# Reecepbcups/celestia-app

Hardware: AMD Instinct MI355X
Metric: ODS→EDS+DAH blocks/sec at k=128 (1/8 GPU); achieved HBM GB/s (higher is better)
Workload: dtype u8; 1 GPU; k128_block_batch: da.ExtendShares+NewDataAvailabilityHeader on 128 independent k=128 blocks per GPU per step (configs[1] per block, batched as configs[2]); k=128, parallelism=blocks x1

## Files before the change

celestia-app_amd/csrc/nmt_dev.h:

```cpp
#pragma once
#include <hip/hip_runtime.h>
#include <stdint.h>

#include "cda_internal.h"
#include "sha256_dev.h"

namespace cda {

__device__ __forceinline__ void load16(const uint4* p, uint32_t* w) {
#pragma unroll
  for (int i = 0; i < 4; i++) {
    uint4 v = p[i];
    w[4 * i + 0] = v.x;
    w[4 * i + 1] = v.y;
    w[4 * i + 2] = v.z;
    w[4 * i + 3] = v.w;
  }
}

__device__ __forceinline__ int ns_cmp(const uint32_t* a, const uint32_t* b) {
#pragma unroll
  for (int i = 0; i < 8; i++) {
    uint32_t x = bswap(a[i]), y = bswap(b[i]);
    if (i == 7) {
      x >>= 24;
      y >>= 24;
    }
    if (x != y) return x < y ? -1 : 1;
  }
  return 0;
}

constexpr uint32_t kParityLeafMid7[8] = {0x1ca5c518, 0x33e5c969, 0xbd2d00ce, 0xa4502bae,
                                         0xce23fa11, 0x90a5b516, 0x5df56d75, 0xf3f677da};
#ifndef CDA_NO_PARITY_MID
#define CDA_NO_PARITY_MID 0
#endif

template <bool PAIRS = true>
__device__ __forceinline__ void leaf_record(const uint4* sh, uint32_t* A, bool q0, uint4* out) {
  uint32_t N[16];
  if (PAIRS) load16(sh + 4, N);
  uint32_t ns[8];
#pragma unroll
  for (int i = 0; i < 8; i++) ns[i] = q0 ? A[i] : 0xFFFFFFFFu;
  uint32_t st[8];
  sha256_init(st);
  uint32_t m[16];
  if (q0) {
    m[0] = be_window(0u, A[0], 3);
#pragma unroll
    for (int i = 1; i < 7; i++) m[i] = be_window(A[i - 1], A[i], 3);
    m[7] = (be_window(A[6], A[7], 3) & 0xFFFF0000u) | (bswap(A[0]) >> 16);
  } else {
    m[0] = 0x00FFFFFFu;
#pragma unroll
    for (int i = 1; i < 7; i++) m[i] = 0xFFFFFFFFu;
    m[7] = 0xFFFF0000u | (bswap(A[0]) >> 16);
  }
#pragma unroll
  for (int i = 8; i < 16; i++) m[i] = be_window(A[i - 8], A[i - 7], 2);
  if (!CDA_NO_PARITY_MID && __all(!q0)) {
    uint32_t mw[16], mid[8];
    mw[0] = 0x00FFFFFFu;
#pragma unroll
    for (int i = 1; i < 7; i++) mw[i] = 0xFFFFFFFFu;
#pragma unroll
    for (int i = 7; i < 16; i++) mw[i] = m[i];
#pragma unroll
    for (int i = 0; i < 8; i++) mid[i] = kParityLeafMid7[i];
    sha256_compress_fenced_from<7, false>(st, mid, mw);
  } else {
    sha256_compress(st, m);
  }
  uint32_t H[8];
#pragma unroll
  for (int i = 0; i < 8; i++) H[i] = A[8 + i];
#pragma unroll 1
  for (int j = 1; j < 8; j++) {
    uint32_t C[16];
    if (!PAIRS) {
      load16(sh + 4 * j, C);
    } else if (j & 1) {
#pragma unroll
      for (int i = 0; i < 16; i++) C[i] = N[i];
    } else {
      load16(sh + 4 * j, C);
      load16(sh + 4 * (j + 1), N);
    }
#pragma unroll
    for (int i = 0; i < 7; i++) m[i] = be_window(H[i], H[i + 1], 2);
    m[7] = be_window(H[7], C[0], 2);
#pragma unroll
    for (int i = 8; i < 16; i++) m[i] = be_window(C[i - 8], C[i - 7], 2);
    sha256_compress(st, m);
#pragma unroll
    for (int i = 0; i < 8; i++) H[i] = C[8 + i];
  }
#pragma unroll
  for (int i = 0; i < 7; i++) m[i] = be_window(H[i], H[i + 1], 2);
  m[7] = be_window(H[7], 0x80u, 2);
#pragma unroll
  for (int i = 8; i < 15; i++) m[i] = 0;
  m[15] = 542u * 8u;
  sha256_compress(st, m);
  uint32_t d[8];
#pragma unroll
  for (int i = 0; i < 8; i++) d[i] = bswap(st[i]);
  uint32_t o[24];
#pragma unroll
  for (int i = 0; i < 7; i++) o[i] = ns[i];
  o[7] = (ns[7] & 0xFFu) | (ns[0] << 8);
#pragma unroll
  for (int i = 8; i < 14; i++) o[i] = le_window(ns[i - 8], ns[i - 7], 3);
  o[14] = (le_window(ns[6], ns[7], 3) & 0xFFFFu) | (d[0] << 16);
#pragma unroll
  for (int i = 15; i < 22; i++) o[i] = le_window(d[i - 15], d[i - 14], 2);
  o[22] = d[7] >> 16;
  o[23] = 0;
#pragma unroll
  for (int i = 0; i < 6; i++) out[i] = make_uint4(o[4 * i], o[4 * i + 1], o[4 * i + 2], o[4 * i + 3]);
}

__device__ __forceinline__ void leaf_cell(const uint8_t* __restrict__ eds, uint4* __restrict__ nodes,
                                          unsigned long long* __restrict__ status, int k, int log2w, uint32_t gid) {
  const int w = 1 << log2w;
  const uint32_t cell = gid & ((1u << (2 * log2w)) - 1);
  const uint32_t blk = gid >> (2 * log2w);
  const int r = (int)(cell >> log2w), c = (int)(cell & (w - 1));
  const bool q0 = (r < k) && (c < k);
  const uint4* sh = reinterpret_cast<const uint4*>(eds + (size_t)gid * CDA_SHARE);

  uint32_t A[16];
  load16(sh, A);
  uint32_t ns[8];
#pragma unroll
  for (int i = 0; i < 8; i++) ns[i] = A[i];

  if (q0) {
    if (c + 1 < k) {
      uint32_t nb[8];
      const uint4* p = reinterpret_cast<const uint4*>(eds + ((size_t)gid + 1) * CDA_SHARE);
      uint4 v0 = p[0], v1 = p[1];
      nb[0] = v0.x; nb[1] = v0.y; nb[2] = v0.z; nb[3] = v0.w;
      nb[4] = v1.x; nb[5] = v1.y; nb[6] = v1.z; nb[7] = v1.w;
      if (ns_cmp(nb, ns) < 0) {
        unsigned long long key = ((unsigned long long)CDA_AXIS_ROW << 40) | ((unsigned long long)r << 20) | (c + 1);
        atomicMin(status + blk, key);
      }
    }
    if (r + 1 < k) {
      uint32_t nb[8];
      const uint4* p = reinterpret_cast<const uint4*>(eds + ((size_t)gid + w) * CDA_SHARE);
      uint4 v0 = p[0], v1 = p[1];
      nb[0] = v0.x; nb[1] = v0.y; nb[2] = v0.z; nb[3] = v0.w;
      nb[4] = v1.x; nb[5] = v1.y; nb[6] = v1.z; nb[7] = v1.w;
      if (ns_cmp(nb, ns) < 0) {
        unsigned long long key = ((unsigned long long)CDA_AXIS_COL << 40) | ((unsigned long long)c << 20) | (r + 1);
        atomicMin(status + blk, key);
      }
    }
  }

  leaf_record(sh, A, q0, nodes + (size_t)gid * 6);
}

__device__ __forceinline__ void ld4(const uint4* p, uint32_t* w) {
#pragma unroll
  for (int i = 0; i < 4; i++) {
    const uint4 v = p[i];
    w[4 * i + 0] = v.x;
    w[4 * i + 1] = v.y;
    w[4 * i + 2] = v.z;
    w[4 * i + 3] = v.w;
  }
}

constexpr uint32_t kParityMid14[8] = {0xa8abd42b, 0x092979bd, 0x8d5926ca, 0x8df58526,
                                      0xa812caa9, 0x7cc8da5d, 0x33a85111, 0x7d669380};
__device__ __forceinline__ void hash_node_mem(const uint4* pl, const uint4* pr, uint4* po, bool store = true,
                                              uint4* ns_lds = nullptr, bool parity = false) {
  uint32_t st[8], m[16];
  sha256_init(st);
  {
    uint32_t L[16];
    ld4(launder(pl), L);
    m[0] = be_window(0x01000000u, L[0], 3);
#pragma unroll
    for (int i = 1; i < 16; i++) m[i] = be_window(L[i - 1], L[i], 3);
    if (ns_lds)
#pragma unroll
      for (int i = 0; i < 4; i++) ns_lds[i] = make_uint4(L[4 * i], L[4 * i + 1], L[4 * i + 2], L[4 * i + 3]);
  }
  if (__all(parity)) {
    uint32_t mw[16];
    mw[0] = 0x01FFFFFFu;
#pragma unroll
    for (int i = 1; i < 14; i++) mw[i] = 0xFFFFFFFFu;
    mw[14] = m[14];
    mw[15] = m[15];
    uint32_t mid[8];
#pragma unroll
    for (int i = 0; i < 8; i++) mid[i] = kParityMid14[i];
    sha256_compress_fenced_from<14>(st, mid, mw);
  } else {
    sha256_compress_fenced(st, m);
  }
  {
    uint32_t L[16], R[16];
    ld4(launder_after(pl, st[0]) + 3, L);
    ld4(launder_after(pr, st[0]), R);
    if (ns_lds)
#pragma unroll
      for (int i = 0; i < 4; i++) ns_lds[4 + i] = make_uint4(R[4 * i], R[4 * i + 1], R[4 * i + 2], R[4 * i + 3]);
#pragma unroll
    for (int i = 0; i < 16; i++) {
      const int wi = 16 + i;
      if (wi <= 21) m[i] = be_window(L[wi - 13], L[wi - 12], 3);
      else if (wi == 22) m[i] = be_window(L[9], L[10], 3) | (R[0] & 0xFFu);
      else m[i] = be_window(R[wi - 23], R[wi - 22], 1);
    }
  }
  sha256_compress_fenced(st, m);
  {
    uint32_t R[16];
    ld4(launder_after(pr, st[0]) + 2, R);
#pragma unroll
    for (int i = 0; i < 16; i++) {
      const int wi = 32 + i;
      if (wi <= 44) m[i] = be_window(R[wi - 31], R[wi - 30], 1);
      else if (wi == 45) m[i] = be_window(R[14], R[15], 1) | 0x00800000u;
      else if (wi == 46) m[i] = 0;
      else m[i] = 181u * 8u;
    }
  }
  sha256_compress_fenced(st, m);

  uint32_t L[16], R[16];
  if (ns_lds) {
    uint32_t z = 0;
    asm volatile("" : "+v"(z) : "v"(st[0]));
    ld4(ns_lds + z, L);
    ld4(ns_lds + z + 4, R);
#pragma unroll
    for (int i = 0; i < 16; i++) asm volatile("" : "+v"(L[i]), "+v"(R[i]));
  } else {
    ld4(launder_after(pl, st[0]), L);
    ld4(launder_after(pr, st[0]), R);
  }
  bool rmin_max = true;
#pragma unroll
  for (int i = 0; i < 7; i++) rmin_max &= (R[i] == 0xFFFFFFFFu);
  rmin_max &= ((R[7] & 0xFFu) == 0xFFu);
  uint32_t S[16];
#pragma unroll
  for (int i = 7; i < 15; i++) S[i] = rmin_max ? L[i] : R[i];
  uint32_t d[8];
#pragma unroll
  for (int i = 0; i < 8; i++) d[i] = bswap(st[i]);
  uint32_t o[24];
#pragma unroll
  for (int i = 0; i < 7; i++) o[i] = L[i];
  o[7] = (L[7] & 0xFFu) | (S[7] & 0xFFFFFF00u);
#pragma unroll
  for (int i = 8; i < 14; i++) o[i] = S[i];
  o[14] = (S[14] & 0xFFFFu) | (d[0] << 16);
#pragma unroll
  for (int i = 15; i < 22; i++) o[i] = le_window(d[i - 15], d[i - 14], 2);
  o[22] = d[7] >> 16;
  o[23] = 0;
  if (store)
#pragma unroll
    for (int i = 0; i < 6; i++) po[i] = make_uint4(o[4 * i], o[4 * i + 1], o[4 * i + 2], o[4 * i + 3]);
}

template <int B>
__device__ __forceinline__ void node_block(const uint32_t (&L)[24], const uint32_t (&R)[24], uint32_t (&m)[16]) {
#pragma unroll
  for (int i = 0; i < 16; i++) {
    const int wi = 16 * B + i;
    if (wi == 0) m[i] = be_window(0x01000000u, L[0], 3);
    else if (wi <= 21) m[i] = be_window(L[wi - 1], L[wi], 3);
    else if (wi == 22) m[i] = be_window(L[21], L[22], 3) | (R[0] & 0xFFu);
    else if (wi <= 44) m[i] = be_window(R[wi - 23], R[wi - 22], 1);
    else if (wi == 45) m[i] = be_window(R[22], R[23], 1) | 0x00800000u;
    else if (wi == 46) m[i] = 0;
    else m[i] = 181u * 8u;
  }
}
__device__ __forceinline__ void node_record(const uint32_t (&L)[24], const uint32_t (&R)[24], const uint32_t (&st)[8],
                                            uint32_t (&o)[24]);

__device__ __forceinline__ void hash_node_regs(const uint32_t (&L)[24], const uint32_t (&R)[24], uint32_t (&o)[24]) {
  uint32_t st[8], m[16];
  sha256_init(st);
  node_block<0>(L, R, m);
  sha256_compress(st, m);
  node_block<1>(L, R, m);
  sha256_compress(st, m);
  node_block<2>(L, R, m);
  sha256_compress(st, m);
  node_record(L, R, st, o);
}
__device__ __forceinline__ void node_record(const uint32_t (&L)[24], const uint32_t (&R)[24], const uint32_t (&st)[8],
                                            uint32_t (&o)[24]) {
  bool rmin_max = true;
#pragma unroll
  for (int i = 0; i < 7; i++) rmin_max &= (R[i] == 0xFFFFFFFFu);
  rmin_max &= ((R[7] & 0xFFu) == 0xFFu);
  uint32_t S[16];
#pragma unroll
  for (int i = 7; i < 15; i++) S[i] = rmin_max ? L[i] : R[i];
  uint32_t d[8];
#pragma unroll
  for (int i = 0; i < 8; i++) d[i] = bswap(st[i]);
#pragma unroll
  for (int i = 0; i < 7; i++) o[i] = L[i];
  o[7] = (L[7] & 0xFFu) | (S[7] & 0xFFFFFF00u);
#pragma unroll
  for (int i = 8; i < 14; i++) o[i] = S[i];
  o[14] = (S[14] & 0xFFFFu) | (d[0] << 16);
#pragma unroll
  for (int i = 15; i < 22; i++) o[i] = le_window(d[i - 15], d[i - 14], 2);
  o[22] = d[7] >> 16;
  o[23] = 0;
}

}
```

celestia-app_amd/csrc/nmt_kernels.hip:

```cpp
#include <hip/hip_runtime.h>
#include <stdint.h>
#include <stdlib.h>

#include <algorithm>
#include <cstdio>
#include <cstdlib>
#include <mutex>
#include <set>

#include "cda_internal.h"
#include "nmt_dev.h"
#include "sha256_dev.h"

namespace cda {

__global__ void __launch_bounds__(256) leaf_hash_kernel(const uint8_t* __restrict__ eds, uint4* __restrict__ nodes,
                                                        unsigned long long* __restrict__ status, int k, int log2w,
                                                        uint32_t total_cells) {
  const uint32_t gid = blockIdx.x * blockDim.x + threadIdx.x;
  if (gid >= total_cells) return;
  leaf_cell(eds, nodes, status, k, log2w, gid);
}

__device__ __forceinline__ void load_node(const uint4* p, uint32_t* n) {
#pragma unroll
  for (int i = 0; i < 6; i++) {
    uint4 v = p[i];
    n[4 * i + 0] = v.x;
    n[4 * i + 1] = v.y;
    n[4 * i + 2] = v.z;
    n[4 * i + 3] = v.w;
  }
}

template <bool FROM_LEAVES>
__global__ void __launch_bounds__(256) nmt_level_kernel(const uint4* __restrict__ in, uint4* __restrict__ out,
                                                        int log2w, int log2n_out, uint32_t total_out) {
  uint32_t gid = blockIdx.x * blockDim.x + threadIdx.x;
  if (gid >= total_out) return;
  const int w = 1 << log2w;
  const uint32_t j = gid & ((1u << log2n_out) - 1);
  const uint32_t tree_g = gid >> log2n_out;
  const uint32_t blk = tree_g >> (log2w + 1);
  const uint32_t tree = tree_g & (2 * w - 1);
  size_t ia, ib;
  if (FROM_LEAVES) {
    const size_t base = (size_t)blk << (2 * log2w);
    if (tree < (uint32_t)w) {
      ia = base + ((size_t)tree << log2w) + 2 * j;
      ib = ia + 1;
    } else {
      const uint32_t col = tree - w;
      ia = base + ((size_t)(2 * j) << log2w) + col;
      ib = ia + w;
    }
  } else {
    ia = ((size_t)tree_g << (log2n_out + 1)) + 2 * j;
    ib = ia + 1;
  }
  hash_node_mem(in + ia * 6, in + ib * 6, out + (size_t)gid * 6);
}

struct LevelDesc {
  uint4* p;
  unsigned long long blk;
  unsigned row0, row_t, row_i, col0, col_t, col_i;
};
struct LevelSet {
  LevelDesc lv[4];
};

__device__ __forceinline__ uint4* level_rec(const LevelDesc& d, unsigned b, bool col, unsigned tree, unsigned i) {
  const unsigned long long off =
      (unsigned long long)b * d.blk + (col ? d.col0 + tree * d.col_t + i * d.col_i : d.row0 + tree * d.row_t + i * d.row_i);
  return d.p + off * 6;
}

__global__ void __launch_bounds__(256) nmt_levels_kernel(LevelSet ls, int log2w, int log2n_out, int M, uint32_t total) {
  const uint32_t gid = blockIdx.x * blockDim.x + threadIdx.x;
  if (gid >= total) return;
  const unsigned w = 1u << log2w;
  const unsigned per_kind = w << log2n_out;
  const unsigned b = gid / (2 * per_kind);
  const unsigned rem = gid - b * 2 * per_kind;
  const bool col = rem >= per_kind;
  const unsigned r2 = col ? rem - per_kind : rem;
  const unsigned tree = col ? (r2 & (w - 1)) : (r2 >> log2n_out);
  const unsigned j = col ? (r2 >> log2w) : (r2 & ((1u << log2n_out) - 1));
  __shared__ uint4 s_ns[256 * 8];
  const unsigned k = w >> 1;
  const int l_in = log2w - log2n_out - M;
  for (int q = 1; q <= M; q++) {
    const unsigned cnt = 1u << (M - q);
    for (unsigned t = 0; t < cnt; t++) {
      const unsigned i = j * cnt + t;
#if CDA_NO_PARITY_MID
      const bool parity = false;
#else
      const bool parity = tree >= k || (i << (l_in + q)) >= k;
#endif
      hash_node_mem(level_rec(ls.lv[q - 1], b, col, tree, 2 * i), level_rec(ls.lv[q - 1], b, col, tree, 2 * i + 1),
                    level_rec(ls.lv[q], b, col, tree, i), true, s_ns + threadIdx.x * 8, parity);
    }
    if (q < M) asm volatile("s_waitcnt vmcnt(0)" ::: "memory");
  }
}

int launch_nmt_trees(const void* d_leaves, void* d_levels, void* d_roots, int k, int nblocks, hipStream_t s,
                     void* prof_ctx) {
  const int w = 2 * k;
  int L = 0;
  while ((1 << L) < w) L++;
  if ((1 << L) != w || L < 1) return -2;
  auto desc = [&](int l) {
    LevelDesc d{};
    const unsigned n = (unsigned)(w >> l);
    if (l == 0) {
      d.p = (uint4*)d_leaves;
      d.blk = (unsigned long long)w * w;
      d.row0 = 0, d.row_t = w, d.row_i = 1, d.col0 = 0, d.col_t = 1, d.col_i = w;
    } else if (l == L) {
      d.p = (uint4*)d_roots;
      d.blk = 2ull * w;
      d.row0 = 0, d.row_t = 1, d.row_i = 0, d.col0 = w, d.col_t = 1, d.col_i = 0;
    } else {
      unsigned long long off = 0;
      for (int q = 1; q < l; q++) off += 2ull * w * (w >> q);
      d.p = (uint4*)d_levels + off * (unsigned long long)nblocks * 6;
      d.blk = 2ull * w * n;
      d.row0 = 0, d.row_t = n, d.row_i = 1, d.col0 = w * n, d.col_t = 1, d.col_i = w;
    }
    return d;
  };
  for (int l_in = 0; l_in < L;) {
    int M = std::min(2, L - l_in);
    if (L - l_in == 3) M = 3;
    LevelSet ls{};
    for (int q = 0; q <= M; q++) ls.lv[q] = desc(l_in + q);
    const int log2n_out = L - (l_in + M);
    const uint32_t total = (uint32_t)nblocks * 2u * ((uint32_t)w << log2n_out);
    {
      ProfScope ps(prof_ctx, l_in == 0 ? "nmt_levels_1" : "nmt_levels", s);
      hipLaunchKernelGGL(nmt_levels_kernel, dim3((total + 255) / 256), dim3(256), 0, s, ls, L, log2n_out, M, total);
    }
    if (hipGetLastError() != hipSuccess) return -1;
    l_in += M;
  }
  return 0;
}

template <int B>
__device__ __forceinline__ void dah_leaf_block(const uint32_t (&L)[24], uint32_t (&m)[16]) {
#pragma unroll
  for (int t = 0; t < 16; t++) {
    const int wi = 16 * B + t;
    if (wi == 0) m[t] = be_window(0u, L[0], 3);
    else if (wi <= 21) m[t] = be_window(L[wi - 1], L[wi], 3);
    else if (wi == 22) m[t] = be_window(L[21], L[22], 3) | 0x80u;
    else if (wi < 31) m[t] = 0;
    else m[t] = 91u * 8u;
  }
}
__device__ __forceinline__ void dah_leaf_digest(const uint32_t (&L)[24], uint32_t (&st)[8]) {
  uint32_t m[16];
  sha256_init(st);
  dah_leaf_block<0>(L, m);
  sha256_compress(st, m);
  dah_leaf_block<1>(L, m);
  sha256_compress(st, m);
}
template <int B>
__device__ __forceinline__ void rfc_node_block(const uint32_t* Ld, const uint32_t* Rd, uint32_t (&m)[16]) {
  if (B == 0) {
    m[0] = 0x01000000u | (Ld[0] >> 8);
#pragma unroll
    for (int t = 1; t < 8; t++) m[t] = (Ld[t - 1] << 24) | (Ld[t] >> 8);
    m[8] = (Ld[7] << 24) | (Rd[0] >> 8);
#pragma unroll
    for (int t = 9; t < 16; t++) m[t] = (Rd[t - 9] << 24) | (Rd[t - 8] >> 8);
  } else {
    m[0] = (Rd[7] << 24) | 0x00800000u;
#pragma unroll
    for (int t = 1; t < 15; t++) m[t] = 0;
    m[15] = 65u * 8u;
  }
}

__device__ __forceinline__ void dah_fold_kw(uint32_t* sdig, int n, uint32_t* out, uint32_t* kw) {
  uint32_t* src = sdig;
  uint32_t* dst = sdig + n * 8;
  for (int cnt = n; cnt > 1;) {
    const int out_cnt = (cnt + 1) >> 1;
    if (out_cnt > 64) {
      for (int i = threadIdx.x; i < out_cnt; i += blockDim.x) {
        uint32_t* o = dst + i * 8;
        const uint32_t* Ld = src + (2 * i) * 8;
        if (2 * i + 1 >= cnt) {
#pragma unroll
          for (int t = 0; t < 8; t++) o[t] = Ld[t];
          continue;
        }
        const uint32_t* Rd = src + (2 * i + 1) * 8;
        uint32_t st[8], m[16];
        sha256_init(st);
        rfc_node_block<0>(Ld, Rd, m);
        sha256_compress(st, m);
        rfc_node_block<1>(Ld, Rd, m);
        sha256_compress(st, m);
#pragma unroll
        for (int t = 0; t < 8; t++) o[t] = st[t];
      }
    } else {
      const int i = threadIdx.x & 63;
      const bool pair = i < out_cnt && 2 * i + 1 < cnt;
      uint32_t st[8];
      if (threadIdx.x < 64) {
        const uint32_t* Ld = src + (2 * i) * 8;
        if (i < out_cnt && !pair)
#pragma unroll
          for (int t = 0; t < 8; t++) dst[i * 8 + t] = Ld[t];
        uint32_t m[16];
        sha256_init(st);
        rfc_node_block<0>(Ld, src + (2 * i + 1) * 8, m);
        sha256_compress(st, m);
      } else if (threadIdx.x < 128) {
        uint32_t m[16];
        rfc_node_block<1>(src + (2 * i) * 8, src + (2 * i + 1) * 8, m);
        sha256_kw_store(m, kw + i * kKwStride);
      }
      __syncthreads();
      if (threadIdx.x < 64) {
        sha256_rounds_kw(st, kw + i * kKwStride);
        if (pair)
#pragma unroll
          for (int t = 0; t < 8; t++) dst[i * 8 + t] = st[t];
      }
    }
    __syncthreads();
    uint32_t* tmp = src;
    src = dst;
    dst = tmp;
    cnt = out_cnt;
  }
  if (threadIdx.x < 8) out[threadIdx.x] = bswap(src[threadIdx.x]);
}

__global__ void __launch_bounds__(256) dah_kernel(const uint4* __restrict__ roots, uint32_t* __restrict__ dah,
                                                  int n) {
  extern __shared__ __attribute__((aligned(16))) uint32_t sdig[];
  const uint4* rb = roots + (size_t)blockIdx.x * n * 6;
  for (int i = threadIdx.x; i < n; i += blockDim.x) {
    uint32_t L[24], st[8];
    load_node(rb + (size_t)i * 6, L);
    dah_leaf_digest(L, st);
#pragma unroll
    for (int t = 0; t < 8; t++) sdig[i * 8 + t] = st[t];
  }
  __syncthreads();
  dah_fold_kw(sdig, n, dah + blockIdx.x * 8, sdig + (n + (n + 1) / 2) * 8);
}

__global__ void __launch_bounds__(256) dah_wide_kernel(const uint4* __restrict__ roots, uint32_t* __restrict__ dah,
                                                       unsigned* __restrict__ done, uint32_t* __restrict__ digests,
                                                       int n, int P) {
  extern __shared__ __attribute__((aligned(16))) uint32_t sdig[];
  __shared__ unsigned last;
  const unsigned b = blockIdx.x / P, part = blockIdx.x % P;
  if (threadIdx.x == 0) last = 0;
  const int i = part * 256 + threadIdx.x;
  if (i < n) {
    uint32_t L[24], st[8];
    load_node(roots + ((size_t)b * n + i) * 6, L);
    dah_leaf_digest(L, st);
    uint4* dg = reinterpret_cast<uint4*>(digests + ((size_t)b * n + i) * 8);
    dg[0] = make_uint4(st[0], st[1], st[2], st[3]);
    dg[1] = make_uint4(st[4], st[5], st[6], st[7]);
  }
  __threadfence();
  __syncthreads();
  if (threadIdx.x == 0) {
    const unsigned prev = __hip_atomic_fetch_add(done + b, 1u, __ATOMIC_ACQ_REL, __HIP_MEMORY_SCOPE_AGENT);
    if (prev == (unsigned)P - 1) last = 1;
  }
  __syncthreads();
  if (!last) return;
  __atomic_thread_fence(__ATOMIC_ACQUIRE);
  const uint4* src = reinterpret_cast<const uint4*>(digests + (size_t)b * n * 8);
  for (int x = threadIdx.x; x < n * 2; x += blockDim.x) reinterpret_cast<uint4*>(sdig)[x] = src[x];
  __syncthreads();
  dah_fold_kw(sdig, n, dah + b * 8, sdig + (n + (n + 1) / 2) * 8);
  if (threadIdx.x == 0) __hip_atomic_store(done + b, 0u, __ATOMIC_RELAXED, __HIP_MEMORY_SCOPE_AGENT);
}

constexpr int kLdsRec = 7;
#ifndef CDA_TREES_TRACE
#define CDA_TREES_TRACE 0
#endif
#if CDA_TREES_TRACE
__device__ unsigned long long* g_trees_trace;
#endif
struct TreesStamps {
  unsigned long long* v;
};
__device__ __forceinline__ void trees_mark(TreesStamps& ts, int slot) {
#if CDA_TREES_TRACE
  if (threadIdx.x == 0) {
    ts.v[2 * slot] = __builtin_amdgcn_s_memrealtime();
    ts.v[2 * slot + 1] = __builtin_amdgcn_s_memtime();
  }
#else
  (void)ts, (void)slot;
#endif
}
__device__ __forceinline__ void trees_flush(const TreesStamps& ts, int lo, int hi) {
#if CDA_TREES_TRACE
  if (threadIdx.x == 0 && g_trees_trace)
    for (int s = lo; s < hi; s++) {
      g_trees_trace[((size_t)blockIdx.x * 32 + s) * 2] = ts.v[2 * s];
      g_trees_trace[((size_t)blockIdx.x * 32 + s) * 2 + 1] = ts.v[2 * s + 1];
    }
#else
  (void)ts, (void)lo, (void)hi;
#endif
}
__device__ __forceinline__ void load_pair(const uint4* in, int i, uint32_t (&L)[24], uint32_t (&R)[24]) {
#pragma unroll
  for (int q = 0; q < 6; q++) {
    const uint4 u = in[(2 * i) * kLdsRec + q], v = in[(2 * i + 1) * kLdsRec + q];
    L[4 * q] = u.x, L[4 * q + 1] = u.y, L[4 * q + 2] = u.z, L[4 * q + 3] = u.w;
    R[4 * q] = v.x, R[4 * q + 1] = v.y, R[4 * q + 2] = v.z, R[4 * q + 3] = v.w;
  }
}
__global__ void __launch_bounds__(256) trees_lds_kernel(const uint4* __restrict__ leaves, uint4* __restrict__ roots,
                                                        uint32_t* __restrict__ dah, unsigned* __restrict__ done,
                                                        uint32_t* __restrict__ digests, int log2w) {
  extern __shared__ __attribute__((aligned(16))) uint4 lds[];
  __shared__ unsigned last;
  const int w = 1 << log2w, n = 2 * w;
  const int half = threadIdx.x >> 7, ht = threadIdx.x & 127;
  const unsigned gtree = blockIdx.x * 2 + half;
  const unsigned b = gtree >> (log2w + 1), tree = gtree & (n - 1);
  const bool col = tree >= (unsigned)w;
  const unsigned t = tree & (w - 1);
  const uint4* lb = leaves + (size_t)b * w * w * 6;
#if CDA_TREES_TRACE
  __shared__ unsigned long long tstamp[64];
  TreesStamps tst{tstamp};
#else
  TreesStamps tst{nullptr};
#endif
  trees_mark(tst, 0);
  if (threadIdx.x == 0) last = 0;
  uint4* A = lds + (size_t)half * (w + w / 2) * kLdsRec;
  uint4* B = A + (size_t)w * kLdsRec;
  uint32_t* kw = reinterpret_cast<uint32_t*>(lds + (size_t)2 * (w + w / 2 + 1) * kLdsRec) + half * 2 * 64 * kKwStride;
  for (int x = ht; x < w * 6; x += 128) {
    const int i = x / 6, q = x - i * 6;
    const size_t rec = col ? ((size_t)i << log2w) + t : ((size_t)t << log2w) + i;
    A[i * kLdsRec + q] = lb[rec * 6 + q];
  }
  __syncthreads();
  trees_mark(tst, 1);
  for (int l = 1; l <= log2w; l++) {
    const uint4* in = (l & 1) ? A : B;
    uint4* out = (l & 1) ? B : A;
    const int nodes = w >> l;
    if (nodes > 64) {
      for (int i = ht; i < nodes; i += 128) {
        uint32_t L[24], R[24], o[24];
        load_pair(in, i, L, R);
        hash_node_regs(L, R, o);
#pragma unroll
        for (int q = 0; q < 6; q++) out[i * kLdsRec + q] = make_uint4(o[4 * q], o[4 * q + 1], o[4 * q + 2], o[4 * q + 3]);
      }
    } else {
      const int i = ht & 63;
      uint32_t L[24], R[24], st[8];
      load_pair(in, i, L, R);
      if (ht < 64) {
        uint32_t m[16];
        sha256_init(st);
        node_block<0>(L, R, m);
        sha256_compress(st, m);
        trees_mark(tst, 2 + 3 * (l - 1));
      } else {
        uint32_t m[16];
        node_block<1>(L, R, m);
        sha256_kw_store(m, kw + i * kKwStride);
        node_block<2>(L, R, m);
        sha256_kw_store(m, kw + (64 + i) * kKwStride);
      }
      __syncthreads();
      trees_mark(tst, 3 + 3 * (l - 1));
      if (ht < 64) {
        sha256_rounds_kw(st, kw + i * kKwStride);
        sha256_rounds_kw(st, kw + (64 + i) * kKwStride);
        uint32_t o[24];
        node_record(L, R, st, o);
        if (i < nodes)
#pragma unroll
          for (int q = 0; q < 6; q++)
            out[i * kLdsRec + q] = make_uint4(o[4 * q], o[4 * q + 1], o[4 * q + 2], o[4 * q + 3]);
      }
    }
    __syncthreads();
// ... 587 lines not shown
```

celestia-app_amd/csrc/sha256_dev.h:

```cpp
#pragma once
#include <hip/hip_runtime.h>
#include <stdint.h>

namespace cda {

__device__ __forceinline__ uint32_t rotr(uint32_t x, int n) { return __builtin_amdgcn_alignbit(x, x, n); }
__device__ __forceinline__ uint32_t xor3(uint32_t a, uint32_t b, uint32_t c) {
  return __builtin_amdgcn_bitop3_b32(a, b, c, 0x96);
}
__device__ __forceinline__ uint32_t ch(uint32_t e, uint32_t f, uint32_t g) {
  return __builtin_amdgcn_bitop3_b32(e, f, g, 0xCA);
}
__device__ __forceinline__ uint32_t maj(uint32_t a, uint32_t b, uint32_t c) {
  return __builtin_amdgcn_bitop3_b32(a, b, c, 0xE8);
}
__device__ __forceinline__ uint32_t bswap(uint32_t x) { return __builtin_bswap32(x); }

__device__ __forceinline__ uint32_t le_window(uint32_t lo, uint32_t hi, int off) {
  return off == 0 ? lo : __builtin_amdgcn_alignbyte(hi, lo, off);
}
__device__ __forceinline__ uint32_t be_window(uint32_t lo, uint32_t hi, int off) {
  const uint32_t sel = (uint32_t)(off + 3) | (uint32_t)(off + 2) << 8 | (uint32_t)(off + 1) << 16 | (uint32_t)off << 24;
  return __builtin_amdgcn_perm(hi, lo, sel);
}

struct K256 {
  static constexpr uint32_t v[64] = {
      0x428a2f98, 0x71374491, 0xb5c0fbcf, 0xe9b5dba5, 0x3956c25b, 0x59f111f1, 0x923f82a4, 0xab1c5ed5,
      0xd807aa98, 0x12835b01, 0x243185be, 0x550c7dc3, 0x72be5d74, 0x80deb1fe, 0x9bdc06a7, 0xc19bf174,
      0xe49b69c1, 0xefbe4786, 0x0fc19dc6, 0x240ca1cc, 0x2de92c6f, 0x4a7484aa, 0x5cb0a9dc, 0x76f988da,
      0x983e5152, 0xa831c66d, 0xb00327c8, 0xbf597fc7, 0xc6e00bf3, 0xd5a79147, 0x06ca6351, 0x14292967,
      0x27b70a85, 0x2e1b2138, 0x4d2c6dfc, 0x53380d13, 0x650a7354, 0x766a0abb, 0x81c2c92e, 0x92722c85,
      0xa2bfe8a1, 0xa81a664b, 0xc24b8b70, 0xc76c51a3, 0xd192e819, 0xd6990624, 0xf40e3585, 0x106aa070,
      0x19a4c116, 0x1e376c08, 0x2748774c, 0x34b0bcb5, 0x391c0cb3, 0x4ed8aa4a, 0x5b9cca4f, 0x682e6ff3,
      0x748f82ee, 0x78a5636f, 0x84c87814, 0x8cc70208, 0x90befffa, 0xa4506ceb, 0xbef9a3f7, 0xc67178f2};
};

__device__ __forceinline__ void sha256_init(uint32_t s[8]) {
  s[0] = 0x6a09e667;
  s[1] = 0xbb67ae85;
  s[2] = 0x3c6ef372;
  s[3] = 0xa54ff53a;
  s[4] = 0x510e527f;
  s[5] = 0x9b05688c;
  s[6] = 0x1f83d9ab;
  s[7] = 0x5be0cd19;
}

__device__ __forceinline__ void sha256_compress(uint32_t s[8], uint32_t w[16]) {
  uint32_t a = s[0], b = s[1], c = s[2], d = s[3], e = s[4], f = s[5], g = s[6], h = s[7];
#pragma unroll
  for (int t = 0; t < 64; t++) {
    uint32_t wt;
    if (t < 16) {
      wt = w[t];
    } else {
      uint32_t w15 = w[(t - 15) & 15], w2 = w[(t - 2) & 15];
      uint32_t s0 = xor3(rotr(w15, 7), rotr(w15, 18), w15 >> 3);
      uint32_t s1 = xor3(rotr(w2, 17), rotr(w2, 19), w2 >> 10);
      wt = w[t & 15] + s0 + w[(t - 7) & 15] + s1;
      w[t & 15] = wt;
    }
    uint32_t t1 = h + xor3(rotr(e, 6), rotr(e, 11), rotr(e, 25)) + ch(e, f, g) + K256::v[t] + wt;
    uint32_t t2 = xor3(rotr(a, 2), rotr(a, 13), rotr(a, 22)) + maj(a, b, c);
    h = g;
    g = f;
    f = e;
    e = d + t1;
    d = c;
    c = b;
    b = a;
    a = t1 + t2;
  }
  s[0] += a;
  s[1] += b;
  s[2] += c;
  s[3] += d;
  s[4] += e;
  s[5] += f;
  s[6] += g;
  s[7] += h;
}

constexpr int kKwStride = 68;
__device__ __forceinline__ void sha256_kw_store(uint32_t (&w)[16], uint32_t* kw) {
#pragma unroll
  for (int t4 = 0; t4 < 16; t4++) {
    uint32_t v[4];
#pragma unroll
    for (int j = 0; j < 4; j++) {
      const int t = 4 * t4 + j;
      uint32_t wt;
      if (t < 16) {
        wt = w[t];
      } else {
        const uint32_t w15 = w[(t - 15) & 15], w2 = w[(t - 2) & 15];
        const uint32_t s0 = xor3(rotr(w15, 7), rotr(w15, 18), w15 >> 3);
        const uint32_t s1 = xor3(rotr(w2, 17), rotr(w2, 19), w2 >> 10);
        wt = w[t & 15] + s0 + w[(t - 7) & 15] + s1;
        w[t & 15] = wt;
      }
      v[j] = wt + K256::v[t];
    }
    reinterpret_cast<uint4*>(kw)[t4] = make_uint4(v[0], v[1], v[2], v[3]);
  }
}
__device__ __forceinline__ void sha256_rounds_kw(uint32_t s[8], const uint32_t* kw) {
  uint32_t a = s[0], b = s[1], c = s[2], d = s[3], e = s[4], f = s[5], g = s[6], h = s[7];
#pragma unroll
  for (int t4 = 0; t4 < 16; t4++) {
    const uint4 q = reinterpret_cast<const uint4*>(kw)[t4];
    const uint32_t kv[4] = {q.x, q.y, q.z, q.w};
#pragma unroll
    for (int j = 0; j < 4; j++) {
      const uint32_t t1 = h + xor3(rotr(e, 6), rotr(e, 11), rotr(e, 25)) + ch(e, f, g) + kv[j];
      const uint32_t t2 = xor3(rotr(a, 2), rotr(a, 13), rotr(a, 22)) + maj(a, b, c);
      h = g;
      g = f;
      f = e;
      e = d + t1;
      d = c;
      c = b;
      b = a;
      a = t1 + t2;
    }
  }
  s[0] += a;
  s[1] += b;
  s[2] += c;
  s[3] += d;
  s[4] += e;
  s[5] += f;
  s[6] += g;
  s[7] += h;
}

template <int N, int SB = 0>
__device__ __forceinline__ void sha256_compress_n(uint32_t (&s)[N][8], uint32_t (&w)[N][16]) {
  uint32_t a[N], b[N], c[N], d[N], e[N], f[N], g[N], h[N];
#pragma unroll
  for (int n = 0; n < N; n++) {
    a[n] = s[n][0]; b[n] = s[n][1]; c[n] = s[n][2]; d[n] = s[n][3];
    e[n] = s[n][4]; f[n] = s[n][5]; g[n] = s[n][6]; h[n] = s[n][7];
  }
#pragma unroll
  for (int t = 0; t < 64; t++) {
#pragma unroll
    for (int n = 0; n < N; n++) {
      uint32_t wt;
      if (t < 16) {
        wt = w[n][t];
      } else {
        uint32_t w15 = w[n][(t - 15) & 15], w2 = w[n][(t - 2) & 15];
        uint32_t s0 = xor3(rotr(w15, 7), rotr(w15, 18), w15 >> 3);
        uint32_t s1 = xor3(rotr(w2, 17), rotr(w2, 19), w2 >> 10);
        wt = w[n][t & 15] + s0 + w[n][(t - 7) & 15] + s1;
        w[n][t & 15] = wt;
      }
      uint32_t t1 = h[n] + xor3(rotr(e[n], 6), rotr(e[n], 11), rotr(e[n], 25)) + ch(e[n], f[n], g[n]) + K256::v[t] + wt;
      uint32_t t2 = xor3(rotr(a[n], 2), rotr(a[n], 13), rotr(a[n], 22)) + maj(a[n], b[n], c[n]);
      h[n] = g[n];
      g[n] = f[n];
      f[n] = e[n];
      e[n] = d[n] + t1;
      d[n] = c[n];
      c[n] = b[n];
      b[n] = a[n];
      a[n] = t1 + t2;
    }
    if (SB > 0 && (t % SB) == SB - 1) __builtin_amdgcn_sched_barrier(0);
  }
#pragma unroll
  for (int n = 0; n < N; n++) {
    s[n][0] += a[n]; s[n][1] += b[n]; s[n][2] += c[n]; s[n][3] += d[n];
    s[n][4] += e[n]; s[n][5] += f[n]; s[n][6] += g[n]; s[n][7] += h[n];
  }
}

__device__ __forceinline__ void sha256_compress_fenced(uint32_t s[8], const uint32_t w[16]) {
  uint32_t S[1][8], W[1][16];
#pragma unroll
  for (int i = 0; i < 8; i++) S[0][i] = s[i];
#pragma unroll
  for (int i = 0; i < 16; i++) W[0][i] = w[i];
  sha256_compress_n<1, 8>(S, W);
#pragma unroll
  for (int i = 0; i < 8; i++) s[i] = S[0][i];
  __builtin_amdgcn_sched_barrier(0);
}

template <int START, bool FENCED = true>
__device__ __forceinline__ void sha256_compress_fenced_from(uint32_t s[8], const uint32_t (&mid)[8],
                                                            uint32_t (&w)[16]) {
  uint32_t a = mid[0], b = mid[1], c = mid[2], d = mid[3], e = mid[4], f = mid[5], g = mid[6], h = mid[7];
#pragma unroll
  for (int t = START; t < 64; t++) {
    uint32_t wt;
    if (t < 16) {
      wt = w[t];
    } else {
      const uint32_t w15 = w[(t - 15) & 15], w2 = w[(t - 2) & 15];
      const uint32_t s0 = xor3(rotr(w15, 7), rotr(w15, 18), w15 >> 3);
      const uint32_t s1 = xor3(rotr(w2, 17), rotr(w2, 19), w2 >> 10);
      wt = w[t & 15] + s0 + w[(t - 7) & 15] + s1;
      w[t & 15] = wt;
    }
    const uint32_t t1 = h + xor3(rotr(e, 6), rotr(e, 11), rotr(e, 25)) + ch(e, f, g) + K256::v[t] + wt;
    const uint32_t t2 = xor3(rotr(a, 2), rotr(a, 13), rotr(a, 22)) + maj(a, b, c);
    h = g;
    g = f;
    f = e;
    e = d + t1;
    d = c;
    c = b;
    b = a;
    a = t1 + t2;
    if (FENCED && (t % 8) == 7) __builtin_amdgcn_sched_barrier(0);
  }
  s[0] += a;
  s[1] += b;
  s[2] += c;
  s[3] += d;
  s[4] += e;
  s[5] += f;
  s[6] += g;
  s[7] += h;
  if (FENCED) __builtin_amdgcn_sched_barrier(0);
}

template <typename T>
__device__ __forceinline__ const T* launder(const T* p) {
  asm volatile("" : "+v"(p));
  return p;
}
template <typename T>
__device__ __forceinline__ const T* launder_after(const T* p, uint32_t after) {
  asm volatile("" : "+v"(p) : "v"(after));
  return p;
}

}
```

Before: 20500 blocks/s.

## Specialize parity-node hashing, remap row threads for uniform parity waves

```diff
diff --git a/celestia-app_amd/csrc/nmt_dev.h b/celestia-app_amd/csrc/nmt_dev.h
--- a/celestia-app_amd/csrc/nmt_dev.h
+++ b/celestia-app_amd/csrc/nmt_dev.h
@@ -60,19 +60,10 @@
   }
 #pragma unroll
   for (int i = 8; i < 16; i++) m[i] = be_window(A[i - 8], A[i - 7], 2);
-  if (!CDA_NO_PARITY_MID && __all(!q0)) {
-    uint32_t mw[16], mid[8];
-    mw[0] = 0x00FFFFFFu;
-#pragma unroll
-    for (int i = 1; i < 7; i++) mw[i] = 0xFFFFFFFFu;
-#pragma unroll
-    for (int i = 7; i < 16; i++) mw[i] = m[i];
-#pragma unroll
-    for (int i = 0; i < 8; i++) mid[i] = kParityLeafMid7[i];
-    sha256_compress_fenced_from<7, false>(st, mid, mw);
-  } else {
-    sha256_compress(st, m);
-  }
+  uint32_t mid[8];
+#pragma unroll
+  for (int i = 0; i < 8; i++) mid[i] = kParityLeafMid7[i];
+  sha256_compress_skip<7>(st, mid, m, !CDA_NO_PARITY_MID && __all(!q0));
   uint32_t H[8];
 #pragma unroll
   for (int i = 0; i < 8; i++) H[i] = A[8 + i];
@@ -176,10 +167,8 @@
   }
 }
 
-constexpr uint32_t kParityMid14[8] = {0xa8abd42b, 0x092979bd, 0x8d5926ca, 0x8df58526,
-                                      0xa812caa9, 0x7cc8da5d, 0x33a85111, 0x7d669380};
 __device__ __forceinline__ void hash_node_mem(const uint4* pl, const uint4* pr, uint4* po, bool store = true,
-                                              uint4* ns_lds = nullptr, bool parity = false) {
+                                              uint4* ns_lds = nullptr) {
   uint32_t st[8], m[16];
   sha256_init(st);
   {
@@ -192,20 +181,7 @@
 #pragma unroll
       for (int i = 0; i < 4; i++) ns_lds[i] = make_uint4(L[4 * i], L[4 * i + 1], L[4 * i + 2], L[4 * i + 3]);
   }
-  if (__all(parity)) {
-    uint32_t mw[16];
-    mw[0] = 0x01FFFFFFu;
-#pragma unroll
-    for (int i = 1; i < 14; i++) mw[i] = 0xFFFFFFFFu;
-    mw[14] = m[14];
-    mw[15] = m[15];
-    uint32_t mid[8];
-#pragma unroll
-    for (int i = 0; i < 8; i++) mid[i] = kParityMid14[i];
-    sha256_compress_fenced_from<14>(st, mid, mw);
-  } else {
-    sha256_compress_fenced(st, m);
-  }
+  sha256_compress_fenced(st, m);
   {
     uint32_t L[16], R[16];
     ld4(launder_after(pl, st[0]) + 3, L);
@@ -265,6 +241,72 @@
 #pragma unroll
   for (int i = 8; i < 14; i++) o[i] = S[i];
   o[14] = (S[14] & 0xFFFFu) | (d[0] << 16);
+#pragma unroll
+  for (int i = 15; i < 22; i++) o[i] = le_window(d[i - 15], d[i - 14], 2);
+  o[22] = d[7] >> 16;
+  o[23] = 0;
+  if (store)
+#pragma unroll
+    for (int i = 0; i < 6; i++) po[i] = make_uint4(o[4 * i], o[4 * i + 1], o[4 * i + 2], o[4 * i + 3]);
+}
+
+constexpr uint32_t kParityMid14[8] = {0xa8abd42b, 0x092979bd, 0x8d5926ca, 0x8df58526,
+                                      0xa812caa9, 0x7cc8da5d, 0x33a85111, 0x7d669380};
+__device__ __forceinline__ void hash_node_parity(const uint4* pl, const uint4* pr, uint4* po, bool store = true) {
+  uint32_t st[8], m[16];
+  sha256_init(st);
+  uint32_t L[12];
+  {
+    const uint4 v = launder(pl)[3];
+    L[3] = v.w;
+    m[0] = 0x01FFFFFFu;
+#pragma unroll
+    for (int i = 1; i < 14; i++) m[i] = 0xFFFFFFFFu;
+    m[14] = be_window(v.y, v.z, 3);
+    m[15] = be_window(v.z, v.w, 3);
+    uint32_t mid[8];
+#pragma unroll
+    for (int i = 0; i < 8; i++) mid[i] = kParityMid14[i];
+    sha256_compress_fenced_from<14>(st, mid, m);
+  }
+  {
+    const uint4* p = launder_after(pl, st[0]) + 3;
+#pragma unroll
+    for (int i = 1; i < 3; i++) {
+      const uint4 v = p[i];
+      L[4 * i] = v.x, L[4 * i + 1] = v.y, L[4 * i + 2] = v.z, L[4 * i + 3] = v.w;
+    }
+  }
+#pragma unroll
+  for (int i = 0; i < 6; i++) m[i] = be_window(L[3 + i], L[4 + i], 3);
+  m[6] = be_window(L[9], L[10], 3) | 0xFFu;
+#pragma unroll
+  for (int i = 7; i < 16; i++) m[i] = 0xFFFFFFFFu;
+  sha256_compress_fenced(st, m);
+  uint32_t R[12];
+  {
+    const uint4* p = launder_after(pr, st[0]) + 3;
+#pragma unroll
+    for (int i = 0; i < 3; i++) {
+      const uint4 v = p[i];
+      R[4 * i] = v.x, R[4 * i + 1] = v.y, R[4 * i + 2] = v.z, R[4 * i + 3] = v.w;
+    }
+  }
+#pragma unroll
+  for (int i = 0; i < 5; i++) m[i] = 0xFFFFFFFFu;
+#pragma unroll
+  for (int i = 5; i < 13; i++) m[i] = be_window(R[i - 3], R[i - 2], 1);
+  m[13] = be_window(R[10], R[11], 1) | 0x00800000u;
+  m[14] = 0;
+  m[15] = 181u * 8u;
+  sha256_compress_fenced(st, m);
+  uint32_t d[8];
+#pragma unroll
+  for (int i = 0; i < 8; i++) d[i] = bswap(st[i]);
+  uint32_t o[24];
+#pragma unroll
+  for (int i = 0; i < 14; i++) o[i] = 0xFFFFFFFFu;
+  o[14] = 0xFFFFu | (d[0] << 16);
 #pragma unroll
   for (int i = 15; i < 22; i++) o[i] = le_window(d[i - 15], d[i - 14], 2);
   o[22] = d[7] >> 16;
diff --git a/celestia-app_amd/csrc/nmt_kernels.hip b/celestia-app_amd/csrc/nmt_kernels.hip
--- a/celestia-app_amd/csrc/nmt_kernels.hip
+++ b/celestia-app_amd/csrc/nmt_kernels.hip
@@ -76,7 +76,8 @@
   return d.p + off * 6;
 }
 
-__global__ void __launch_bounds__(256) nmt_levels_kernel(LevelSet ls, int log2w, int log2n_out, int M, uint32_t total) {
+__global__ void __launch_bounds__(256) __attribute__((amdgpu_waves_per_eu(4)))
+nmt_levels_kernel(LevelSet ls, int log2w, int log2n_out, int M, uint32_t total) {
   const uint32_t gid = blockIdx.x * blockDim.x + threadIdx.x;
   if (gid >= total) return;
   const unsigned w = 1u << log2w;
@@ -85,8 +86,23 @@
   const unsigned rem = gid - b * 2 * per_kind;
   const bool col = rem >= per_kind;
   const unsigned r2 = col ? rem - per_kind : rem;
-  const unsigned tree = col ? (r2 & (w - 1)) : (r2 >> log2n_out);
-  const unsigned j = col ? (r2 >> log2w) : (r2 & ((1u << log2n_out) - 1));
+  unsigned tree, j;
+  if (col) {
+    tree = r2 & (w - 1);
+    j = r2 >> log2w;
+  } else if (log2n_out == 0) {
+    tree = r2;
+    j = 0;
+  } else {
+    const int log2h = log2n_out - 1;
+    const int T = min(max(6 - log2h, 0), log2w);
+    const unsigned jl = r2 & ((1u << log2h) - 1);
+    const unsigned tl = (r2 >> log2h) & ((1u << T) - 1);
+    const unsigned half = (r2 >> (log2h + T)) & 1u;
+    const unsigned th = r2 >> (log2h + T + 1);
+    tree = (th << T) | tl;
+    j = (half << log2h) | jl;
+  }
   __shared__ uint4 s_ns[256 * 8];
   const unsigned k = w >> 1;
   const int l_in = log2w - log2n_out - M;
@@ -99,8 +115,11 @@
 #else
       const bool parity = tree >= k || (i << (l_in + q)) >= k;
 #endif
-      hash_node_mem(level_rec(ls.lv[q - 1], b, col, tree, 2 * i), level_rec(ls.lv[q - 1], b, col, tree, 2 * i + 1),
-                    level_rec(ls.lv[q], b, col, tree, i), true, s_ns + threadIdx.x * 8, parity);
+      const uint4* pl = level_rec(ls.lv[q - 1], b, col, tree, 2 * i);
+      const uint4* pr = level_rec(ls.lv[q - 1], b, col, tree, 2 * i + 1);
+      uint4* po = level_rec(ls.lv[q], b, col, tree, i);
+      if (__all(parity)) hash_node_parity(pl, pr, po);
+      else hash_node_mem(pl, pr, po, true, s_ns + threadIdx.x * 8);
     }
     if (q < M) asm volatile("s_waitcnt vmcnt(0)" ::: "memory");
   }
diff --git a/celestia-app_amd/csrc/sha256_dev.h b/celestia-app_amd/csrc/sha256_dev.h
--- a/celestia-app_amd/csrc/sha256_dev.h
+++ b/celestia-app_amd/csrc/sha256_dev.h
@@ -228,6 +228,60 @@
   if (FENCED) __builtin_amdgcn_sched_barrier(0);
 }
 
+template <int START>
+__device__ __forceinline__ void sha256_compress_skip(uint32_t s[8], const uint32_t (&mid)[8], uint32_t (&w)[16],
+                                                     bool skip) {
+  uint32_t a = s[0], b = s[1], c = s[2], d = s[3], e = s[4], f = s[5], g = s[6], h = s[7];
+  if (skip) {
+    a = mid[0], b = mid[1], c = mid[2], d = mid[3], e = mid[4], f = mid[5], g = mid[6], h = mid[7];
+  } else {
+#pragma unroll
+    for (int t = 0; t < START; t++) {
+      const uint32_t t1 = h + xor3(rotr(e, 6), rotr(e, 11), rotr(e, 25)) + ch(e, f, g) + K256::v[t] + w[t];
+      const uint32_t t2 = xor3(rotr(a, 2), rotr(a, 13), rotr(a, 22)) + maj(a, b, c);
+      h = g;
+      g = f;
+      f = e;
+      e = d + t1;
+      d = c;
+      c = b;
+      b = a;
+      a = t1 + t2;
+    }
+  }
+#pragma unroll
+  for (int t = START; t < 64; t++) {
+    uint32_t wt;
+    if (t < 16) {
+      wt = w[t];
+    } else {
+      const uint32_t w15 = w[(t - 15) & 15], w2 = w[(t - 2) & 15];
+      const uint32_t s0 = xor3(rotr(w15, 7), rotr(w15, 18), w15 >> 3);
+      const uint32_t s1 = xor3(rotr(w2, 17), rotr(w2, 19), w2 >> 10);
+      wt = w[t & 15] + s0 + w[(t - 7) & 15] + s1;
+      w[t & 15] = wt;
+    }
+    const uint32_t t1 = h + xor3(rotr(e, 6), rotr(e, 11), rotr(e, 25)) + ch(e, f, g) + K256::v[t] + wt;
+    const uint32_t t2 = xor3(rotr(a, 2), rotr(a, 13), rotr(a, 22)) + maj(a, b, c);
+    h = g;
+    g = f;
+    f = e;
+    e = d + t1;
+    d = c;
+    c = b;
+    b = a;
+    a = t1 + t2;
+  }
+  s[0] += a;
+  s[1] += b;
+  s[2] += c;
+  s[3] += d;
+  s[4] += e;
+  s[5] += f;
+  s[6] += g;
+  s[7] += h;
+}
+
 template <typename T>
 __device__ __forceinline__ const T* launder(const T* p) {
   asm volatile("" : "+v"(p));
```

Measured after the change: 20850 blocks/s (median of 6 runs). +1.7%, better.
